# ginevracoal/robustBNNs

Measured on AMD Instinct MI355X. Metric: attack-samples/sec (test_pts x posterior_samples x PGD_iters), higher is better.
Workload: dtype f32 (full-width operands as three f16 pieces: 6 exact f16 MFMA product terms per fp32 product, f32 accumulate)

## Files before the change

robustbnns_amd/csrc/rbnn_triple.hip:

```cpp
#include "rbnn_common.hpp"
#include <algorithm>
#include <cstdlib>

namespace {

__device__ __forceinline__ void split3(float v, _Float16& p0, _Float16& p1, _Float16& p2) {
    p0 = (_Float16)v;
    float r = v - (float)p0;
    p1 = (_Float16)r;
    r -= (float)p1;
    p2 = (_Float16)r;
}

#ifndef RBNN_X3_PAIR_NOP
#define RBNN_X3_PAIR_NOP 0
#endif
#if RBNN_X3_PAIR_NOP
#define RBNN_X3_PAIR_PAD "\n\ts_nop 1"
#else
#define RBNN_X3_PAIR_PAD ""
#endif
#define RBNN_X3_PAIR_BODY \
    "v_bfe_i32 %[me], %[mw], %[b0], 1\n\t" \
    "v_bfe_i32 %[mo], %[mw], %[b1], 1\n\t" \
// ... 208 lines not shown
                if (k == 0 && ht + 1 < HTW) {
                    a0n = *(const f16x8*)(Wt + (ht + 1) * 3072);
                    a1n = *(const f16x8*)(Wt + (ht + 1) * 3072 + 1024);
                    a2n = *(const f16x8*)(Wt + (ht + 1) * 3072 + 2048);
                }
            }
            a0 = a0n; a1 = a1n; a2 = a2n;
        }
        {
            __builtin_amdgcn_sched_group_barrier(0x100, 3 * NTW + 3, 0);
#pragma unroll
            for (int ht = 0; ht < HTW; ++ht) {
                __builtin_amdgcn_sched_group_barrier(0x008, 3 * NTW, 0);
                if (ht + 1 < HTW) __builtin_amdgcn_sched_group_barrier(0x100, 3, 0);
                __builtin_amdgcn_sched_group_barrier(0x008, 3 * NTW, 0);
            }
        }
        if (!(RBNN_ABL & 2)) ring_wait_barrier<0>();
        const int hc0 = ch * BH;
        kt = wrap ? 0 : kt + 1;
        ch = wrap ? ch + 1 : ch;
        if (!wrap) continue;

        if (RBNN_ABL & 8) {
            float t = 0.f;
#pragma unroll
            for (int ht = 0; ht < HTW; ++ht)
#pragma unroll
                for (int nt = 0; nt < NTW; ++nt) { t += acc[ht][nt][0] + acc[ht][nt][1] + acc[ht][nt][2] + acc[ht][nt][3]; acc[ht][nt] = (f32x4){0.f, 0.f, 0.f, 0.f}; }
            if (t == 12345.678f) a.P[tid] = t;
            continue;
        }
        const int hw0 = hc0 + (wave_h * HTW) * 16;
        unsigned mine[NTW];
#pragma unroll
        for (int nt = 0; nt < NTW; ++nt) mine[nt] = 0u;
#pragma unroll
        for (int ht = 0; ht < HTW; ++ht) {
            const int hrow = hw0 + ht * 16 + 4 * lg;
            const f32x4 bias = *(const f32x4*)(a.b + (long long)sw * a.H + hrow);
            f32x4 w2f = (f32x4){0.f, 0.f, 0.f, 0.f};
            if (LAYER2 && li < a.C) w2f = *(const f32x4*)(a.W2 + ((long long)sw * a.C + li) * a.H + hrow);
#pragma unroll
            for (int nt = 0; nt < NTW; ++nt) {
                const int n = n0 + (wave_n * NTW + nt) * 16 + li;
                f32x4 v = acc[ht][nt] * out_scale + bias, hv;
                acc[ht][nt] = (f32x4){0.f, 0.f, 0.f, 0.f};
                unsigned bits = 0;
#pragma unroll
                for (int r = 0; r < 4; ++r) {
                    bits |= (v[r] > 0.f ? 1u : 0u) << r;
                    hv[r] = act_fwd<ACT>(v[r]);
                }
                if (BITMASK) {
                    unsigned part = bits << (16 * (ht & 1) + 4 * lg);
                    part |= __shfl_xor(part, 16);
                    part |= __shfl_xor(part, 32);
                    if (lg == (ht >> 1)) mine[nt] |= part;
                }
                if (!BITMASK && a.dact && n < a.N) {
                    f32x4 dv;
#pragma unroll
                    for (int r = 0; r < 4; ++r) dv[r] = act_grad_from_value<ACT>(hv[r]);
                    *(f32x4*)(a.dact + ((long long)s * a.N + n) * a.H + hrow) = dv;
                }
                if (LAYER2) {
#pragma unroll
                    for (int r = 0; r < 4; ++r) zacc[nt] = MFMA16(w2f[r], hv[r], zacc[nt]);
                } else {
#ifdef RBNN_X3_L1_ABL_NOSTORE
                    if (n < a.N && hv[0] == 1.2345e-30f) {
#else
                    if (n < a.N) {
#endif
                        const long long blk = ((long long)s * HW + (hrow >> 5)) * ((a.N + 15) >> 4) + (n >> 4);
#ifdef RBNN_X3_L1_ABL_SMALL
                        char* const row = a.hid + ((blk * 2048) & 0xFFC00) + (n & 15) * 128 + ((hrow >> 4) & 1) * 64 + lg * 16;
#else
                        char* const row = a.hid + blk * 2048 + (n & 15) * 128 + ((hrow >> 4) & 1) * 64 + lg * 16;
#endif
                        *(f32x4*)row = hv * hid_scale;
                    }
                }
            }
        }
        if (BITMASK && a.mask) {
#pragma unroll
            for (int nt = 0; nt < NTW; ++nt) {
                const int n = n0 + (wave_n * NTW + nt) * 16 + li;
                if (lg < HTW / 2 && n < a.N) a.mask[((long long)s * HW + (hw0 >> 5) + lg) * mask_ld(a.N) + n] = mine[nt];
            }
        }
    }
    if (RBNN_ABL & 2) ring_wait_barrier<0>();

    if (!LAYER2) return;
#pragma unroll
    for (int nt = 0; nt < NTW; ++nt)
        *(f32x4*)(zred + (wave_h * BN + (wave_n * NTW + nt) * 16 + li) * 16 + 4 * lg) = zacc[nt];
    __syncthreads();
    if (tid < BN) {
        const int n = n0 + tid;
        float z[16];
#pragma unroll
        for (int q = 0; q < 4; ++q) {
            f32x4 sum = *(const f32x4*)(zred + tid * 16 + 4 * q);
#pragma unroll
            for (int w = 1; w < WH; ++w) sum += *(const f32x4*)(zred + (w * BN + tid) * 16 + 4 * q);
#pragma unroll
            for (int r = 0; r < 4; ++r) z[4 * q + r] = sum[r];
        }
        float m = -INFINITY;
#pragma unroll
        for (int c = 0; c < 16; ++c) {
            if (c < a.C) { z[c] += a.b2[(long long)sw * a.C + c]; m = fmaxf(m, z[c]); }
            else z[c] = 0.f;
        }
        if (a.out_kind == RBNN_OUT_PROBS) {
            float den = 0.f;
#pragma unroll
            for (int c = 0; c < 16; ++c) if (c < a.C) { z[c] = expf(z[c] - m); den += z[c]; }
#pragma unroll
            for (int c = 0; c < 16; ++c) if (c < a.C) z[c] = z[c] / den;
        }
        if (n < a.N) {
            float* const dst = a.P + ((long long)s * a.N + n) * RBNN_CPAD;
#pragma unroll
            for (int q = 0; q < 4; ++q) *(f32x4*)(dst + 4 * q) = (f32x4){z[4 * q], z[4 * q + 1], z[4 * q + 2], z[4 * q + 3]};
        }
    }
}

template <int ACT, int WH, int HTW, int WN, int NTW, bool LAYER2, bool XF32>
int launch_forward_x3_cfg(FwdX3Args a, hipStream_t st) {
    constexpr int BH = WH * HTW * 16, BN = WN * NTW * 16;
    constexpr int LDSB = 2 * 3 * (BH + BN) * 64;
    static_assert(LDSB <= 160 * 1024, "LDS");
    a.NT = (a.N + BN - 1) / BN;
    auto kern = fc_forward_x3_kernel<ACT, WH, HTW, WN, NTW, LAYER2, XF32>;
    static unsigned long long attr_done = 0;
    if (!ensure_dynamic_lds((const void*)kern, LDSB, attr_done)) return RBNN_ERR_LAUNCH;
    const int grid = grid_for_items((long long)a.NT * a.S);
    hipLaunchKernelGGL(kern, dim3(grid), dim3(64 * WH * WN), LDSB, st, a);
    return launch_status();
}

template <int ACT, bool LAYER2, bool XF32>
int launch_forward_x3_act(const FwdX3Args& a, hipStream_t st) {
    if (a.H % 256 == 0) return launch_forward_x3_cfg<ACT, 4, 4, 2, 4, LAYER2, XF32>(a, st);
    if (a.H % 128 == 0) return launch_forward_x3_cfg<ACT, 2, 4, 2, 4, LAYER2, XF32>(a, st);
    return RBNN_ERR_UNSUPPORTED;
}

template <bool LAYER2, bool XF32 = false>
int launch_forward_x3(int act, const FwdX3Args& a, hipStream_t st) {
    switch (act) {
#ifndef RBNN_FAST_BUILD
        case RBNN_ACT_RELU:  return launch_forward_x3_act<RBNN_ACT_RELU, LAYER2, XF32>(a, st);
#endif
        case RBNN_ACT_LEAKY: return launch_forward_x3_act<RBNN_ACT_LEAKY, LAYER2, XF32>(a, st);
#ifndef RBNN_FAST_BUILD
        case RBNN_ACT_SIGM:  return launch_forward_x3_act<RBNN_ACT_SIGM, LAYER2, XF32>(a, st);
        case RBNN_ACT_TANH:  return launch_forward_x3_act<RBNN_ACT_TANH, LAYER2, XF32>(a, st);
#endif
    }
    return RBNN_ERR_UNSUPPORTED;
}

__global__ void triple_cols_kernel(const float* __restrict__ W, long long n_mats, int rows, int cols, int ld_src, float scale,
                                   uint4* __restrict__ dst, int ld_dst) {
    const long long i = (long long)blockIdx.x * blockDim.x + threadIdx.x;
    const int HB = rows / 32;
    if (i >= n_mats * HB * 4 * ld_dst) return;
    const int d = (int)(i % ld_dst);
    const int lg = (int)((i / ld_dst) % 4);
    const long long mh = i / (4LL * ld_dst);
    const long long m = mh / HB;
    const int hb = (int)(mh % HB);
    union { f16x8 v; uint4 u; } o[3];
#pragma unroll
    for (int j = 0; j < 8; ++j) {
        const int h = 32 * hb + 16 * (j >> 2) + 4 * lg + (j & 3);
        const float v = (d < cols) ? W[(m * rows + h) * ld_src + d] * scale : 0.f;
        _Float16 a, b, c;
        split3(v, a, b, c);
        o[0].v[j] = a; o[1].v[j] = b; o[2].v[j] = c;
    }
    const long long base = ((mh * 4 + lg) * 3) * ld_dst;
    dst[base + d] = o[0].u;
    dst[base + ld_dst + d] = o[1].u;
    dst[base + 2 * ld_dst + d] = o[2].u;
}

__global__ void triple_w2gen_kernel(const float* __restrict__ W2, int n_mats, int C, int H, float scale, uint4* __restrict__ dst) {
    const long long i = (long long)blockIdx.x * blockDim.x + threadIdx.x;
    if (i >= (long long)n_mats * (H / 16) * 128) return;
    const int lane = (int)(i & 63), li = lane & 15, lg = lane >> 4, k = (int)((i >> 6) & 1);
    const int t = (int)((i >> 7) % (H / 16));
    const long long m = (i >> 7) / (H / 16);
    _Float16 w[3][10];
#pragma unroll
    for (int c = 0; c < 10; ++c) {
        const float v = (c < C) ? W2[(m * C + c) * H + 16 * t + li] * scale : 0.f;
        split3(v, w[0][c], w[1][c], w[2][c]);
    }
    union { f16x8 v; uint4 u; } o;
    const _Float16 z = (_Float16)0.f;
    if (lg < 3) {
        const int piece = (k == 0) ? (lg == 2 ? 1 : 0) : (lg == 0 ? 1 : (lg == 1 ? 0 : 2));
#pragma unroll
        for (int j = 0; j < 8; ++j) o.v[j] = piece == 0 ? w[0][j] : (piece == 1 ? w[1][j] : w[2][j]);
    } else if (k == 0) {
        o.v[0] = w[0][8]; o.v[1] = w[0][9]; o.v[2] = w[0][8]; o.v[3] = w[0][9];
        o.v[4] = w[0][8]; o.v[5] = w[0][9]; o.v[6] = w[1][8]; o.v[7] = w[1][9];
    } else {
        o.v[0] = w[2][8]; o.v[1] = w[2][9]; o.v[2] = w[1][8]; o.v[3] = w[1][9];
        o.v[4] = z; o.v[5] = z; o.v[6] = z; o.v[7] = z;
    }
    dst[i] = o.u;
}

__host__ __device__ __forceinline__ int dz_swz3(long long n) { return (int)((0 - (n >> 2)) & 3); }

__global__ void __launch_bounds__(256) triple_dz_kernel(const float* __restrict__ dZ, int S, int N, long long N_pad, int C,
                                                        uint4* __restrict__ dst, float* __restrict__ gscale) {
    __shared__ float red[16][17];
    const int p = threadIdx.x & 15, q = threadIdx.x >> 4;
    const long long n = (long long)blockIdx.x * 16 + p;
    float m = 0.f;
    if (n < N)
        for (int s = q; s < S; s += 16) {
            const float* const src = dZ + ((long long)s * N + n) * RBNN_CPAD;
#pragma unroll
            for (int k = 0; k < 3; ++k) {
                const f32x4 v = *(const f32x4*)(src + 4 * k);
#pragma unroll
                for (int r = 0; r < 4; ++r) if (4 * k + r < C) m = fmaxf(m, fabsf(v[r]));
            }
        }
    red[q][p] = m;
    __syncthreads();
    m = 0.f;
#pragma unroll
    for (int i = 0; i < 16; ++i) m = fmaxf(m, red[i][p]);
    int e = 0;
    if (m > 0.f && m < INFINITY) e = min(13 - ilogbf(m), 120);
    if (q == 0) gscale[n] = ldexpf(1.f, -e);
    const int sw = dz_swz3(n);
    for (int s = q; s < S; s += 16) {
        _Float16 d[3][10];
        float v[12];
        if (n < N) {
            const float* const src = dZ + ((long long)s * N + n) * RBNN_CPAD;
#pragma unroll
            for (int k = 0; k < 3; ++k) {
                const f32x4 t = *(const f32x4*)(src + 4 * k);
#pragma unroll
                for (int r = 0; r < 4; ++r) v[4 * k + r] = t[r];
            }
        }
#pragma unroll
        for (int c = 0; c < 10; ++c) {
            const float x = (n < N && c < C) ? ldexpf(v[c], e) : 0.f;
            split3(x, d[0][c], d[1][c], d[2][c]);
        }
        uint4* const o = dst + ((long long)s * N_pad + n) * 4;
#pragma unroll
        for (int ch = 0; ch < 3; ++ch) {
            union { f16x8 v; uint4 u; } w;
#pragma unroll
            for (int j = 0; j < 8; ++j) w.v[j] = d[ch][j];
            o[ch ^ sw] = w.u;
        }
        union { f16x8 v; uint4 u; } t;
        t.v[0] = d[0][8]; t.v[1] = d[0][9]; t.v[2] = d[1][8]; t.v[3] = d[1][9];
        t.v[4] = d[2][8]; t.v[5] = d[2][9]; t.v[6] = d[0][8]; t.v[7] = d[0][9];
        o[3 ^ sw] = t.u;
    }
}

template <int MODE>
__device__ __forceinline__ void tail_dz(const float* __restrict__ prow, const float (&gmean)[16], int y, int C, float inv_S, float (&out)[16]) {
    float p[16], g[16];
#pragma unroll
    for (int q = 0; q < 4; ++q) {
        const f32x4 v = *(const f32x4*)(prow + 4 * q);
#pragma unroll
        for (int r = 0; r < 4; ++r) p[4 * q + r] = v[r];
    }
    if (MODE == RBNN_LOSS_PER_SAMPLE) {
        ce_softmax_grad<16>(p, C, y, inv_S, g);
    } else {
#pragma unroll
        for (int c = 0; c < 16; ++c) g[c] = gmean[c];
    }
    if (MODE == RBNN_LOSS_MEAN_LOGIT) {
#pragma unroll
        for (int c = 0; c < 16; ++c) out[c] = g[c];
    } else {
        softmax_backward<16>(g, p, C, out);
    }
}

template <int MODE>
__global__ void __launch_bounds__(256) step_tail_x3_kernel(const float* __restrict__ P, const int* __restrict__ labels, int S, float inv_S, int N,
                                                           long long N_pad, int C, float* __restrict__ Psum_out, int ldo,
                                                           uint4* __restrict__ dst, float* __restrict__ gscale) {
    __shared__ float red[16][17];
    __shared__ float psum[16][16];
    const int p = threadIdx.x & 15, q = threadIdx.x >> 4;
    const long long n = (long long)blockIdx.x * 16 + p;
    if (MODE != RBNN_LOSS_PER_SAMPLE) {
        if (q < 4) {
            f32x4 sum = (f32x4){0.f, 0.f, 0.f, 0.f};
            if (n < N)
                for (int s = 0; s < S; ++s) sum += *(const f32x4*)(P + ((long long)s * N + n) * RBNN_CPAD + 4 * q);
#pragma unroll
            for (int r = 0; r < 4; ++r) {
                psum[p][4 * q + r] = sum[r];
                if (Psum_out && n < N && 4 * q + r < C) Psum_out[n * ldo + 4 * q + r] = sum[r];
            }
        }
        __syncthreads();
    }
    const int y = (n < N) ? labels[n] : 0;
    float gmean[16];
    if (MODE != RBNN_LOSS_PER_SAMPLE) {
        float t[16];
#pragma unroll
        for (int c = 0; c < 16; ++c) t[c] = (c < C) ? psum[p][c] * inv_S : 0.f;
        ce_softmax_grad<16>(t, C, y, inv_S, gmean);
    } else {
#pragma unroll
        for (int c = 0; c < 16; ++c) gmean[c] = 0.f;
    }
    float m = 0.f;
    if (n < N)
        for (int s = q; s < S; s += 16) {
            float dz[16];
            tail_dz<MODE>(P + ((long long)s * N + n) * RBNN_CPAD, gmean, y, C, inv_S, dz);
#pragma unroll
            for (int c = 0; c < 12; ++c) if (c < C) m = fmaxf(m, fabsf(dz[c]));
        }
    red[q][p] = m;
    __syncthreads();
    m = 0.f;
#pragma unroll
    for (int i = 0; i < 16; ++i) m = fmaxf(m, red[i][p]);
    int e = 0;
    if (m > 0.f && m < INFINITY) e = min(13 - ilogbf(m), 120);
    if (q == 0) gscale[n] = ldexpf(1.f, -e);
    const int sw = dz_swz3(n);
    for (int s = q; s < S; s += 16) {
        _Float16 d[3][10];
        float dz[16];
#pragma unroll
        for (int c = 0; c < 16; ++c) dz[c] = 0.f;
        if (n < N) tail_dz<MODE>(P + ((long long)s * N + n) * RBNN_CPAD, gmean, y, C, inv_S, dz);
#pragma unroll
        for (int c = 0; c < 10; ++c) {
            const float x = (n < N && c < C) ? ldexpf(dz[c], e) : 0.f;
            split3(x, d[0][c], d[1][c], d[2][c]);
        }
        uint4* const o = dst + ((long long)s * N_pad + n) * 4;
#pragma unroll
        for (int ch = 0; ch < 3; ++ch) {
            union { f16x8 v; uint4 u; } w;
#pragma unroll
            for (int j = 0; j < 8; ++j) w.v[j] = d[ch][j];
            o[ch ^ sw] = w.u;
        }
        union { f16x8 v; uint4 u; } t;
        t.v[0] = d[0][8]; t.v[1] = d[0][9]; t.v[2] = d[1][8]; t.v[3] = d[1][9];
        t.v[4] = d[2][8]; t.v[5] = d[2][9]; t.v[6] = d[0][8]; t.v[7] = d[0][9];
        o[3 ^ sw] = t.u;
    }
}

__global__ void __launch_bounds__(256) attack_step_x3_kernel(float* __restrict__ X, const float* __restrict__ X0, int ldx, const float* __restrict__ G,
                                                             int K, long long slab_stride, int ldg, const float* __restrict__ alpha, float alpha_scalar,
                                                             float eps, int project, long long N, int D, const rbnn_dev_scale* __restrict__ ds,
                                                             uint4* __restrict__ dst, int groups) {
    const long long i = (long long)blockIdx.x * blockDim.x + threadIdx.x;
    if (i >= N * groups) return;
    const long long n = i / groups;
    const int gq = (int)(i % groups), d0 = 8 * gq;
    const float scale = ds->scale;
    float xn[8];
#pragma unroll
    for (int j = 0; j < 8; ++j) xn[j] = 0.f;
    if (d0 < D) {
        const float step = alpha ? alpha[n] : alpha_scalar;
#pragma unroll
        for (int h = 0; h < 2; ++h) {
            const int d = d0 + 4 * h;
            if (d < D) {
                f32x4 g = *(const f32x4*)(G + n * ldg + d);
                for (int k = 1; k < K; ++k) g += *(const f32x4*)(G + k * slab_stride + n * ldg + d);
                const f32x4 x = *(const f32x4*)(X + n * ldx + d);
                f32x4 x0 = x, out;
                if (project) x0 = *(const f32x4*)(X0 + n * ldx + d);
#pragma unroll
                for (int r = 0; r < 4; ++r) {
                    const float sgn = (g[r] > 0.f) ? 1.f : ((g[r] < 0.f) ? -1.f : 0.f);
                    float pert = x[r] + step * sgn;
                    if (project) pert = x0[r] + fminf(fmaxf(pert - x0[r], -eps), eps);
                    out[r] = fminf(fmaxf(pert, 0.f), 1.f);
                    xn[4 * h + r] = out[r];
                }
                *(f32x4*)(X + n * ldx + d) = out;
            }
        }
    }
    union { f16x8 v; uint4 u; } o[3];
#pragma unroll
    for (int j = 0; j < 8; ++j) {
        const float v = (d0 + j < D) ? xn[j] * scale : 0.f;
        _Float16 a, b, c;
        split3(v, a, b, c);
        o[0].v[j] = a; o[1].v[j] = b; o[2].v[j] = c;
    }
    uint4* const out = dst + (((n >> 4) * (groups >> 2) + (gq >> 2)) * 192 + (n & 15) * 4 + (gq & 3));
    out[0] = o[0].u; out[64] = o[1].u; out[128] = o[2].u;
}

#define GEN_Q3 (-17)

struct GradX3Args {
    const char* dzg;  long long n_pad;  const float* gscale;  const uint32_t* mask;
    const char* W1c;  int ldc;
    const char* W2g;
    int H;  int HW;  const int* sidx;  int S;  int chunk;  int nchunks;
    int N;  int NT;  int ND;  int Dt;
    float* out;  int ldo;  float out_scale;
    const uint32_t* omask;  int OHW;
    const float* amem;
    const float* dact;  const float* odact;
};
enum { X3_FC = 0, X3_FC2_STEP1 = 1, X3_FC2_STEP2 = 2 };

template <int ACT, int TD, int MODE>
__global__ void __launch_bounds__(256, 2) fc_grad_x3_kernel(const GradX3Args a) {
    constexpr int NW = 4;
    constexpr bool GEN = MODE != X3_FC2_STEP2;
    constexpr bool BITMASK = (ACT == RBNN_ACT_RELU || ACT == RBNN_ACT_LEAKY);
    constexpr bool STREAM = !GEN || !BITMASK;
    constexpr int NTW = 16 / NW, BM = 256, LD = TD * 16;
    constexpr int W1B = 12 * LD * 16;
    constexpr int NPIECE = W1B / 1024, PPW = (NPIECE + NW - 1) / NW;
    constexpr int BUFB = W1B + 4096 + 1024;
    constexpr int DZB = BM * 64;
    static_assert(W1B % 1024 == 0, "whole DMA pieces");
    extern __shared__ __attribute__((aligned(16))) float lds[];
    char* const ldsb = (char*)lds;
    char* const dzl = ldsb + 2 * BUFB;

    int id;
    if (!item_of_block(blockIdx.x, a.NT * a.ND * a.nchunks, id)) return;
    int ntile, dg, ch;
    grad_item(id, a.NT, a.ND, STREAM, ntile, dg, ch);
    const int tid = threadIdx.x, lane = tid & 63, li = lane & 15, lg = lane >> 4;
    const int wave = __builtin_amdgcn_readfirstlane(tid >> 6);
    const int nb = ntile * BM + wave * (NTW * 16);
    const int dc0 = dg * LD;
    const int Dp = a.Dt * 16;
    const int ntd = min(TD, a.Dt - dg * TD);
    const int s_begin = ch * a.chunk, s_end = min(a.S, s_begin + a.chunk);
    const int HS = a.H / 32, nst = (s_end - s_begin) * HS;

    unsigned goff[PPW];
#pragma unroll
    for (int i = 0; i < PPW; ++i) {
        const int f = (wave + NW * i) * 1024 + lane * 16, seg = f / (LD * 16), d = (f % (LD * 16)) >> 4;
        goff[i] = (unsigned)(seg * a.ldc + min(dc0 + d, a.ldc - 1)) * 16u;
    }
    const unsigned loff = (unsigned)lane * 16u;

    f32x4 acc[NTW][TD];
#pragma unroll
    for (int nt = 0; nt < NTW; ++nt)
#pragma unroll
        for (int dt = 0; dt < TD; ++dt) acc[nt][dt] = (f32x4){0.f, 0.f, 0.f, 0.f};

    auto dz_issue = [&](int s) {
        const char* const src = a.dzg + ((long long)s * a.n_pad + nb) * 64;
#pragma unroll
        for (int j = 0; j < NTW; ++j) glds16((const float*)(src + j * 1024 + loff), (float*)(dzl + wave * (NTW * 1024) + j * 1024));
    };
    constexpr int NDMA = GEN ? (BITMASK ? PPW + 2 : PPW + 1) : PPW;
    struct StageSrc { const char* W; const char* G; const char* M; char* B; };
    auto stage_src = [&](int st, int buf) {
        const int si = st / HS, hb = st % HS, s = s_begin + si;
        const int sw = a.sidx ? a.sidx[s] : s;
        StageSrc r;
        r.W = a.W1c + ((long long)sw * HS + hb) * 12 * a.ldc * 16;
        r.G = a.W2g + ((long long)sw * (a.H / 16) + 2 * hb) * 2048 + wave * 1024;
        r.M = (const char*)(a.mask + ((long long)s * a.HW + hb) * a.n_pad + ntile * BM);
        r.B = ldsb + buf * BUFB;
        return r;
    };
    auto issue_piece = [&](const StageSrc& q, int i) {
        if (i < PPW) {
            if (wave + NW * i < NPIECE) glds16((const float*)(q.W + goff[i < PPW ? i : 0]), (float*)(q.B + (wave + NW * i) * 1024));
        } else if (i == PPW) {
            glds16((const float*)(q.G + loff), (float*)(q.B + W1B + wave * 1024));
        } else if (BITMASK && i == PPW + 1) {
            if (wave == NW - 1) glds16((const float*)(q.M + loff), (float*)(q.B + W1B + 4096));
        }
    };

    if (GEN) dz_issue(s_begin);
    {
        const StageSrc q = stage_src(0, 0);
#pragma unroll
        for (int i = 0; i < NDMA; ++i) issue_piece(q, i);
    }
    f32x4 am[STREAM ? NTW : 1][2];
    auto load_a = [&](int st) {
        const int s = s_begin + st / HS, h0 = (st % HS) * 32;
        const float* const base = GEN ? a.dact : a.amem;
#pragma unroll
        for (int nt = 0; nt < (STREAM ? NTW : 0); ++nt) {
            const int n = min(nb + nt * 16 + li, a.N - 1);
            const float* const src = base + ((long long)s * a.N + n) * a.H + h0 + 4 * lg;
            am[nt][0] = *(const f32x4*)src;
            am[nt][1] = *(const f32x4*)(src + 16);
        }
    };
    if (STREAM) load_a(0);
    ring_wait_barrier<0>();
    const float c_pos = ldexpf(1.f, GEN_Q3);
    const unsigned cp_bits = __float_as_uint(c_pos);
    const unsigned cn_bits = (ACT == RBNN_ACT_RELU) ? 0u : __float_as_uint(LEAKY_SLOPE * ldexpf(1.f, GEN_Q3));
    const int dzc1 = (lg == 2 ? 0 : lg), dzc2 = (lg == 0 ? 1 : (lg == 1 ? 2 : (lg == 2 ? 0 : 3)));
    const int sz = dz_swz3(li);
    const char* const dzw = dzl + wave * (NTW * 1024) + li * 64;
    f16x8 da0[NTW], da1[NTW], da2[NTW];
    for (int st = 0; st < nst; ++st) {
        const int buf = st & 1, hb = st % HS;
        const bool more = !(RBNN_ABL & 1) && st + 1 < nst;
        const StageSrc q = stage_src(more ? st + 1 : st, buf ^ 1);
        const char* const B = ldsb + buf * BUFB;
        const bool gen_on = GEN && (!(RBNN_ABL & 16) || st == 0);
        if (!GEN) {
#pragma unroll
            for (int nt = 0; nt < (GEN ? 0 : NTW); ++nt) {
                union { f16x8 v; unsigned u[4]; } o0, o1, o2;
#pragma unroll
                for (int t = 0; t < 2; ++t) {
                    split3_plain_pair(am[nt][t][0], am[nt][t][1], 1.f, o0.u[2 * t], o1.u[2 * t], o2.u[2 * t]);
                    split3_plain_pair(am[nt][t][2], am[nt][t][3], 1.f, o0.u[2 * t + 1], o1.u[2 * t + 1], o2.u[2 * t + 1]);
                }
                da0[nt] = o0.v; da1[nt] = o1.v; da2[nt] = o2.v;
            }
        }
        if (more) {
#pragma unroll
            for (int i = 0; i < NDMA; ++i) issue_piece(q, i);
        }
        f32x4 dm[(GEN && STREAM) ? NTW : 1][2];
        if (GEN && STREAM) {
#pragma unroll
            for (int nt = 0; nt < ((GEN && STREAM) ? NTW : 0); ++nt) { dm[nt][0] = am[nt][0] * c_pos; dm[nt][1] = am[nt][1] * c_pos; }
        }
        if (STREAM && st + 1 < nst) load_a(st + 1);

        if (gen_on) {
            const f16x8 w00 = *(const f16x8*)(B + W1B + lane * 16);
            const f16x8 w01 = *(const f16x8*)(B + W1B + 1024 + lane * 16);
            const f16x8 w10 = *(const f16x8*)(B + W1B + 2048 + lane * 16);
            const f16x8 w11 = *(const f16x8*)(B + W1B + 3072 + lane * 16);
            const unsigned* const Mk = (const unsigned*)(B + W1B + 4096) + wave * (NTW * 16) + li;
#pragma unroll
            for (int nt = 0; nt < NTW; ++nt) {
                const f16x8 dz1 = *(const f16x8*)(dzw + nt * 1024 + ((dzc1 ^ sz) * 16));
                const f16x8 dz2 = *(const f16x8*)(dzw + nt * 1024 + ((dzc2 ^ sz) * 16));
                const f32x4 z = (f32x4){0.f, 0.f, 0.f, 0.f};
                const f32x4 g0 = MFMA_H(w01, dz2, MFMA_H(w00, dz1, z)), g1 = MFMA_H(w11, dz2, MFMA_H(w10, dz1, z));
                union { f16x8 v; unsigned u[4]; } o0, o1, o2;
                if constexpr (BITMASK) {
                    const unsigned mw = Mk[nt * 16] >> (4 * lg);
                    split3_pair<0, true>(g0[0], g0[1], mw, cp_bits, cn_bits, 1.f, o0.u[0], o1.u[0], o2.u[0]);
                    split3_pair<2, false>(g0[2], g0[3], mw, cp_bits, cn_bits, 1.f, o0.u[1], o1.u[1], o2.u[1]);
                    split3_pair<16, true>(g1[0], g1[1], mw, cp_bits, cn_bits, 1.f, o0.u[2], o1.u[2], o2.u[2]);
                    split3_pair<18, false>(g1[2], g1[3], mw, cp_bits, cn_bits, 1.f, o0.u[3], o1.u[3], o2.u[3]);
                } else {
                    constexpr int q = (GEN && STREAM) ? 1 : 0;
                    split3_pair_m<true>(g0[0], g0[1], dm[q * nt][0][0], dm[q * nt][0][1], 1.f, o0.u[0], o1.u[0], o2.u[0]);
                    split3_pair_m<false>(g0[2], g0[3], dm[q * nt][0][2], dm[q * nt][0][3], 1.f, o0.u[1], o1.u[1], o2.u[1]);
                    split3_pair_m<true>(g1[0], g1[1], dm[q * nt][1][0], dm[q * nt][1][1], 1.f, o0.u[2], o1.u[2], o2.u[2]);
                    split3_pair_m<false>(g1[2], g1[3], dm[q * nt][1][2], dm[q * nt][1][3], 1.f, o0.u[3], o1.u[3], o2.u[3]);
                }
                da0[nt] = o0.v; da1[nt] = o1.v; da2[nt] = o2.v;
            }
        }
        if (GEN && !(RBNN_ABL & 1) && hb == HS - 1 && st + 1 < nst) {
            asm volatile("" ::: "memory");
            __builtin_amdgcn_s_waitcnt(0xC07F);
            asm volatile("" ::: "memory");
            dz_issue(s_begin + st / HS + 1);
        }
        const char* const Bw = B + (lg * 3 * LD + li) * 16;
        f16x8 bb[2][3];
        bb[0][0] = *(const f16x8*)(Bw); bb[0][1] = *(const f16x8*)(Bw + LD * 16); bb[0][2] = *(const f16x8*)(Bw + 2 * LD * 16);
#pragma unroll
        for (int dt = 0; dt < TD; ++dt) {
            if (dt < ntd) {
                f16x8 (&bc)[3] = bb[dt & 1];
                if (dt + 1 < TD) {
                    f16x8 (&bn)[3] = bb[(dt + 1) & 1];
                    bn[0] = *(const f16x8*)(Bw + (dt + 1) * 256);
                    bn[1] = *(const f16x8*)(Bw + LD * 16 + (dt + 1) * 256);
                    bn[2] = *(const f16x8*)(Bw + 2 * LD * 16 + (dt + 1) * 256);
                }
#pragma unroll
                for (int nt = 0; nt < NTW; ++nt) acc[nt][dt] = MFMA_H(da0[nt], bc[2], acc[nt][dt]);
#pragma unroll
                for (int nt = 0; nt < NTW; ++nt) acc[nt][dt] = MFMA_H(da2[nt], bc[0], acc[nt][dt]);
#pragma unroll
                for (int nt = 0; nt < NTW; ++nt) acc[nt][dt] = MFMA_H(da1[nt], bc[1], acc[nt][dt]);
#pragma unroll
                for (int nt = 0; nt < NTW; ++nt) acc[nt][dt] = MFMA_H(da1[nt], bc[0], acc[nt][dt]);
#pragma unroll
                for (int nt = 0; nt < NTW; ++nt) acc[nt][dt] = MFMA_H(da0[nt], bc[1], acc[nt][dt]);
#pragma unroll
                for (int nt = 0; nt < NTW; ++nt) acc[nt][dt] = MFMA_H(da0[nt], bc[0], acc[nt][dt]);
            }
        }
        if (!(RBNN_ABL & 2)) ring_wait_barrier<0>();
    }
    if (RBNN_ABL & 2) ring_wait_barrier<0>();

    if (RBNN_ABL & 8) {
        float t = 0.f;
#pragma unroll
        for (int nt = 0; nt < NTW; ++nt)
#pragma unroll
            for (int dt = 0; dt < TD; ++dt) t += acc[nt][dt][0] + acc[nt][dt][1] + acc[nt][dt][2] + acc[nt][dt][3];
        if (t == 12345.678f) a.out[tid] = t;
        return;
    }
    constexpr int LDW = LD + 4, C4 = LD / 4, E4 = 16 * C4;
    static_assert(NW * 16 * LDW * 4 <= 2 * BUFB + DZB, "the waves' transposition tiles fit the loop buffers");
    float* const tw = (float*)ldsb + wave * (16 * LDW);
#pragma unroll
    for (int nt = 0; nt < NTW; ++nt) {
#pragma unroll
        for (int r = 0; r < 4; ++r) {
            const int n = nb + nt * 16 + 4 * lg + r;
            const float gs = (MODE == X3_FC2_STEP1) ? a.out_scale : (n < a.N ? a.gscale[n] : 0.f) * a.out_scale;
#pragma unroll
            for (int dt = 0; dt < TD; ++dt) tw[(4 * lg + r) * LDW + dt * 16 + li] = acc[nt][dt][r] * gs;
        }
#pragma unroll
        for (int i = 0; i < (E4 + 63) / 64; ++i) {
            const int e4 = i * 64 + lane, row = e4 / C4, c4 = e4 - row * C4;
            const int n = nb + nt * 16 + row, d = dc0 + 4 * c4;
            if (e4 < E4 && n < a.N && d < Dp) {
                f32x4 v = *(const f32x4*)(tw + row * LDW + 4 * c4);
                if (MODE == X3_FC2_STEP1) {
                    if (BITMASK) {
                        const unsigned w = a.omask[((long long)ch * a.OHW + (d >> 5)) * a.n_pad + n] >> (d & 31);
#pragma unroll
                        for (int k = 0; k < 4; ++k) v[k] = ((w >> k) & 1u) ? v[k] : (ACT == RBNN_ACT_RELU ? 0.f : v[k] * LEAKY_SLOPE);
                    } else {
                        v *= *(const f32x4*)(a.odact + ((long long)ch * a.N + n) * a.ldo + d);
                    }
                }
                *(f32x4*)(a.out + ((long long)ch * a.N + n) * a.ldo + d) = v;
            }
        }
    }
}

template <int ACT, int TD, int MODE>
int launch_grad_x3_cfg(GradX3Args a, hipStream_t st) {
    constexpr int LDSB = 2 * (12 * TD * 16 * 16 + 5120) + 256 * 64;
    static_assert(2 * LDSB <= 160 * 1024, "two blocks per CU");
    a.NT = (a.N + 255) / 256;
    a.ND = (a.Dt + TD - 1) / TD;
    auto kern = fc_grad_x3_kernel<ACT, TD, MODE>;
    static unsigned long long attr_done = 0;
    if (!ensure_dynamic_lds((const void*)kern, LDSB, attr_done)) return RBNN_ERR_LAUNCH;
    const int grid = grid_for_items((long long)a.NT * a.ND * a.nchunks);
    hipLaunchKernelGGL(kern, dim3(grid), dim3(256), LDSB, st, a);
    return launch_status();
}

inline bool x3_grad_td9() {
    static const bool on = [] { const char* e = getenv("RBNN_X3_GRAD_TD9"); return !e || e[0] != '0'; }();
    return on;
}

template <int ACT, int TD, int MODE>
bool x3_grad_two_blocks() {
    static int ok[64] = {0};
    int dev = 0;
    if (hipGetDevice(&dev) != hipSuccess || dev < 0 || dev >= 64) return false;
    if (!ok[dev]) {
        constexpr int LDSB = 2 * (12 * TD * 16 * 16 + 5120) + 256 * 64;
        auto kern = fc_grad_x3_kernel<ACT, TD, MODE>;
        static unsigned long long attr_done = 0;
        int nb = 0;
        const bool fine = ensure_dynamic_lds((const void*)kern, LDSB, attr_done) &&
                          hipOccupancyMaxActiveBlocksPerMultiprocessor(&nb, kern, 256, LDSB) == hipSuccess && nb >= 2;
        ok[dev] = fine ? 1 : 2;
    }
    return ok[dev] == 1;
}

template <int ACT, int MODE>
int launch_grad_x3(const GradX3Args& a, hipStream_t st) {
    if constexpr (MODE == X3_FC && (ACT == RBNN_ACT_RELU || ACT == RBNN_ACT_LEAKY)) {
        if (x3_grad_td9() && (a.Dt + 8) / 9 < (a.Dt + 6) / 7 && x3_grad_two_blocks<ACT, 9, MODE>()) return launch_grad_x3_cfg<ACT, 9, MODE>(a, st);
    }
    if constexpr (MODE != X3_FC2_STEP2 && (ACT == RBNN_ACT_RELU || ACT == RBNN_ACT_LEAKY)) {
        if (x3_grad_td9() && (a.Dt + 7) / 8 < (a.Dt + 6) / 7 && x3_grad_two_blocks<ACT, 8, MODE>()) return launch_grad_x3_cfg<ACT, 8, MODE>(a, st);
    }
    if ((a.Dt + 6) / 7 < (a.Dt + 3) / 4) return launch_grad_x3_cfg<ACT, 7, MODE>(a, st);
    return launch_grad_x3_cfg<ACT, 4, MODE>(a, st);
}

template <int MODE>
int launch_grad_x3_act(int act, const GradX3Args& a, hipStream_t st) {
#ifndef RBNN_FAST_BUILD
    if (act == RBNN_ACT_RELU) return launch_grad_x3<RBNN_ACT_RELU, MODE>(a, st);
    if (act == RBNN_ACT_SIGM || act == RBNN_ACT_TANH) return launch_grad_x3<RBNN_ACT_SIGM, MODE>(a, st);
#endif
    return launch_grad_x3<RBNN_ACT_LEAKY, MODE>(a, st);
}

}

extern "C" {

static int triple_rows_launch(const float* src, int64_t rows, int32_t cols, int32_t ld_src, int32_t scale_exp,
                              const rbnn_dev_scale* dev_scale, void* dst, int32_t ld_dst, void* stream, int grouped) {
    if (!src || !dst) return RBNN_ERR_NULL;
    if (rows < 1 || cols < 1 || ld_src < cols || ld_dst < cols || (ld_dst & 31)) return RBNN_ERR_SHAPE;
    if (scale_exp < -100 || scale_exp > 100) return RBNN_ERR_SHAPE;
    if (!aligned16(dst)) return RBNN_ERR_ALIGN;
    const int groups = ld_dst / 8;
    const long long total = (long long)rows * groups;
    hipLaunchKernelGGL(triple_rows_kernel, dim3((unsigned)((total + 255) / 256)), dim3(256), 0, (hipStream_t)stream,
                       src, (long long)rows, cols, ld_src, ldexpf(1.f, scale_exp), dev_scale, (uint4*)dst, groups, grouped);
    return launch_status();
}

int rbnn_triple_rows(const float* src, int64_t rows, int32_t cols, int32_t ld_src, int32_t scale_exp,
                     const rbnn_dev_scale* dev_scale, void* dst, int32_t ld_dst, void* stream) {
    return triple_rows_launch(src, rows, cols, ld_src, scale_exp, dev_scale, dst, ld_dst, stream, 0);
}

int rbnn_triple_rows_grouped(const float* src, int64_t rows, int32_t cols, int32_t ld_src, int32_t scale_exp,
                             const rbnn_dev_scale* dev_scale, void* dst, int32_t ld_dst, void* stream) {
    return triple_rows_launch(src, rows, cols, ld_src, scale_exp, dev_scale, dst, ld_dst, stream, 1);
}

int rbnn_triple_cols(const float* W, int64_t n_mats, int32_t rows, int32_t cols, int32_t ld_src, int32_t scale_exp,
                     void* dst, int32_t ld_dst, void* stream) {
    if (!W || !dst) return RBNN_ERR_NULL;
    if (n_mats < 1 || rows < 32 || (rows & 31) || cols < 1 || ld_src < cols || ld_dst < cols || (ld_dst & 15)) return RBNN_ERR_SHAPE;
    if (scale_exp < -100 || scale_exp > 100) return RBNN_ERR_SHAPE;
    if (!aligned16(dst)) return RBNN_ERR_ALIGN;
    const long long total = (long long)n_mats * (rows / 32) * 4 * ld_dst;
    hipLaunchKernelGGL(triple_cols_kernel, dim3((unsigned)((total + 255) / 256)), dim3(256), 0, (hipStream_t)stream,
                       W, (long long)n_mats, rows, cols, ld_src, ldexpf(1.f, scale_exp), (uint4*)dst, ld_dst);
    return launch_status();
}

int rbnn_triple_w2gen(const float* W2, int32_t n_mats, int32_t C, int32_t H, int32_t scale_exp, void* dst, void* stream) {
    if (!W2 || !dst) return RBNN_ERR_NULL;
    if (n_mats < 1 || C < 1 || C > 10 || H < 16 || (H & 15)) return RBNN_ERR_SHAPE;
    if (scale_exp < -100 || scale_exp > 100) return RBNN_ERR_SHAPE;
    if (!aligned16(dst)) return RBNN_ERR_ALIGN;
    const long long total = (long long)n_mats * (H / 16) * 128;
    hipLaunchKernelGGL(triple_w2gen_kernel, dim3((unsigned)((total + 255) / 256)), dim3(256), 0, (hipStream_t)stream,
                       W2, n_mats, C, H, ldexpf(1.f, scale_exp), (uint4*)dst);
    return launch_status();
}

int rbnn_triple_workspace_query(const rbnn_posterior* net, const rbnn_triple_images* tp, int32_t N, int32_t S,
                                rbnn_triple_workspace_sizes* out) {
    if (!net || !tp || !out) return RBNN_ERR_NULL;
    if (N < 1 || S < 1 || tp->ld_rows < net->in_features || (tp->ld_rows & 31)) return RBNN_ERR_SHAPE;
    rbnn_triple_workspace_sizes z = {};
    z.X_triple = (size_t)((N + 15) / 16 * 16) * tp->ld_rows * 6;
    z.dZ_gen = (size_t)S * mask_ld(N) * 64;
    z.g_scale = (size_t)mask_ld(N) * sizeof(float);
    z.hid_triple = net->arch == RBNN_ARCH_FC2 ? (size_t)S * ((N + 15) / 16 * 16) * net->hidden * 4 : 0;
    *out = z;
    return RBNN_OK;
}

int rbnn_fc_forward_triple(const rbnn_posterior* net, const rbnn_triple_images* tp, const rbnn_triple_workspace* tws,
                           int32_t x_exp, const rbnn_dev_scale* dev_scales, int32_t N, const int32_t* sidx, int32_t S,
                           int32_t out_kind, const rbnn_workspace* ws, void* stream) {
    if (!net || !tp || !tws || !tws->X_triple || !ws || !ws->P || !tp->W1_rows) return RBNN_ERR_NULL;
    if (!net->b1 || !net->W2 || !net->b2) return RBNN_ERR_NULL;
    if (net->arch != RBNN_ARCH_FC && net->arch != RBNN_ARCH_FC2) return RBNN_ERR_UNSUPPORTED;
    if (net->activation < RBNN_ACT_RELU || net->activation > RBNN_ACT_TANH) return RBNN_ERR_UNSUPPORTED;
    const bool fc2 = net->arch == RBNN_ARCH_FC2, bm = net->activation == RBNN_ACT_RELU || net->activation == RBNN_ACT_LEAKY;
    const int H = net->hidden, ld = tp->ld_rows;
    if (H < 128 || (H % 128) || ld < net->in_features || (ld & 31)) return RBNN_ERR_SHAPE;
    if (net->n_classes < 1 || net->n_classes > RBNN_CPAD || N < 1 || S < 1) return RBNN_ERR_SHAPE;
    if ((long long)H * ld * 6 >= (1LL << 32) || ((long long)N + 15) * ld * 6 >= (1LL << 32) || ((long long)N + 15) * H * 6 >= (1LL << 32)) return RBNN_ERR_SHAPE;
    if (out_kind != RBNN_OUT_PROBS && out_kind != RBNN_OUT_LOGITS) return RBNN_ERR_UNSUPPORTED;
    if (!aligned16(tws->X_triple) || !aligned16(tp->W1_rows) || !aligned16(ws->P) || !aligned16(net->b1) || !aligned16(net->W2)) return RBNN_ERR_ALIGN;
    if (fc2 && (!tp->Wm_rows || !net->bm || !tws->hid_triple || (bm ? !ws->mask2 : !ws->dact2))) return RBNN_ERR_NULL;
    if (fc2 && (!aligned16(tp->Wm_rows) || !aligned16(tws->hid_triple) || !aligned16(net->bm))) return RBNN_ERR_ALIGN;
    hipStream_t st = (hipStream_t)stream;
    FwdX3Args a = {};
    a.X = (const char*)tws->X_triple; a.ldx = ld; a.N = N; a.x_sample_bytes = 0; a.x_group_bytes = (unsigned)(ld / 32) * 3072u; a.x_stage_bytes = 3072u;
    a.W = (const char*)tp->W1_rows; a.w_sample_bytes = (long long)H * ld * 6; a.ldw = ld; a.KT = ld / 32;
    a.b = net->b1; a.W2 = net->W2; a.b2 = net->b2; a.C = net->n_classes; a.H = H;
    a.sidx = sidx; a.S = S; a.out_scale = ldexpf(1.f, -((dev_scales ? 0 : x_exp) + tp->w1_exp)); a.x_ds = dev_scales;
    a.P = ws->P; a.mask = ws->mask1; a.dact = ws->dact1; a.out_kind = out_kind;
    if (!fc2) return launch_forward_x3<true>(net->activation, a, st);
    a.hid = (char*)tws->hid_triple; a.hid_scale = ldexpf(1.f, tp->h1_exp); a.hid_ds = dev_scales ? dev_scales + 1 : nullptr;
    int rc = launch_forward_x3<false>(net->activation, a, st);
    if (rc) return rc;
    FwdX3Args b = a;
    const int NG = (N + 15) / 16;
    b.X = (const char*)tws->hid_triple; b.ldx = H; b.x_sample_bytes = (long long)NG * 16 * H * 4; b.x_group_bytes = 2048u; b.x_stage_bytes = (unsigned)NG * 2048u;
    b.W = (const char*)tp->Wm_rows; b.w_sample_bytes = (long long)H * H * 6; b.ldw = H; b.KT = H / 32;
    b.b = net->bm; b.out_scale = ldexpf(1.f, -((dev_scales ? 0 : tp->h1_exp) + tp->wm_exp));
    b.x_ds = dev_scales ? dev_scales + 1 : nullptr; b.hid_ds = nullptr;
    b.mask = ws->mask2; b.dact = ws->dact2; b.hid = nullptr;
    return launch_forward_x3<true, true>(net->activation, b, st);
}

int rbnn_step_tail_triple(int32_t mode, const float* P, const int32_t* labels, int32_t S, float inv_S, int32_t N, int32_t C, float* Psum_out,
                          int32_t ldo, const rbnn_triple_workspace* tws, void* stream) {
    if (!P || !labels || !tws || !tws->dZ_gen || !tws->g_scale) return RBNN_ERR_NULL;
    if (mode != RBNN_LOSS_MEAN_PROB && mode != RBNN_LOSS_PER_SAMPLE && mode != RBNN_LOSS_MEAN_LOGIT) return RBNN_ERR_UNSUPPORTED;
    if (S < 1 || N < 1 || C < 1 || C > 10 || (Psum_out && ldo < C)) return RBNN_ERR_SHAPE;
    if (!aligned16(P) || !aligned16(tws->dZ_gen)) return RBNN_ERR_ALIGN;
    const long long n_pad = mask_ld(N);
    const dim3 grid((unsigned)(n_pad / 16)), block(256);
    hipStream_t st = (hipStream_t)stream;
    if (mode == RBNN_LOSS_MEAN_PROB)
        hipLaunchKernelGGL(step_tail_x3_kernel<RBNN_LOSS_MEAN_PROB>, grid, block, 0, st, P, labels, S, inv_S, N, n_pad, C, Psum_out, ldo, (uint4*)tws->dZ_gen, tws->g_scale);
    else if (mode == RBNN_LOSS_PER_SAMPLE)
        hipLaunchKernelGGL(step_tail_x3_kernel<RBNN_LOSS_PER_SAMPLE>, grid, block, 0, st, P, labels, S, inv_S, N, n_pad, C, Psum_out, ldo, (uint4*)tws->dZ_gen, tws->g_scale);
    else
        hipLaunchKernelGGL(step_tail_x3_kernel<RBNN_LOSS_MEAN_LOGIT>, grid, block, 0, st, P, labels, S, inv_S, N, n_pad, C, Psum_out, ldo, (uint4*)tws->dZ_gen, tws->g_scale);
    return launch_status();
}

int rbnn_attack_step_triple(float* X, const float* X0, int32_t ldx, const float* G, int32_t K, size_t slab_stride, int32_t ldg, const float* alpha,
                            float alpha_scalar, float eps, int32_t project, int32_t N, int32_t D, const rbnn_dev_scale* dev_scale, void* X_triple,
                            int32_t ld_rows, void* stream) {
    if (!X || !G || (project && !X0) || !dev_scale || !X_triple) return RBNN_ERR_NULL;
    if (N < 1 || D < 1 || ldx < D || ldg < D || K < 1 || ld_rows < D || (ld_rows & 31)) return RBNN_ERR_SHAPE;
    if ((D & 3) || (ldx & 3) || (ldg & 3) || (slab_stride & 3)) return RBNN_ERR_SHAPE;
    if (!aligned16(X) || !aligned16(G) || (project && !aligned16(X0)) || !aligned16(X_triple)) return RBNN_ERR_ALIGN;
    const int groups = ld_rows / 8;
    const long long total = (long long)N * groups;
    hipLaunchKernelGGL(attack_step_x3_kernel, dim3((unsigned)((total + 255) / 256)), dim3(256), 0, (hipStream_t)stream,
                       X, X0, ldx, G, K, (long long)slab_stride, ldg, alpha, alpha_scalar, eps, project, (long long)N, D, dev_scale, (uint4*)X_triple, groups);
    return launch_status();
}

int rbnn_fc_input_grad_triple(const rbnn_posterior* net, const rbnn_triple_images* tp, const int32_t* sidx, int32_t S,
                              int32_t N, int32_t chunk, const rbnn_workspace* ws, const rbnn_triple_workspace* tws,
                              int32_t* n_slabs_out, void* stream) {
    if (!net || !tp || !ws || !tws || !ws->slabs) return RBNN_ERR_NULL;
    if (!tp->W1_cols || !tp->W2_gen || !tws->dZ_gen || !tws->g_scale) return RBNN_ERR_NULL;
    if (net->arch != RBNN_ARCH_FC && net->arch != RBNN_ARCH_FC2) return RBNN_ERR_UNSUPPORTED;
    if (net->activation < RBNN_ACT_RELU || net->activation > RBNN_ACT_TANH) return RBNN_ERR_UNSUPPORTED;
    const bool fc2 = net->arch == RBNN_ARCH_FC2, bm = net->activation == RBNN_ACT_RELU || net->activation == RBNN_ACT_LEAKY;
    if (bm ? !ws->mask1 : !ws->dact1) return RBNN_ERR_NULL;
    if (fc2 && (bm ? !ws->mask2 : !ws->dact2)) return RBNN_ERR_NULL;
    const int H = net->hidden, Dp = net->in_stride, C = net->n_classes;
    if (H < 128 || (H % 128) || C < 1 || C > 10 || N < 1 || S < 1) return RBNN_ERR_SHAPE;
    if (tp->ld_cols != Dp || (Dp & 15)) return RBNN_ERR_SHAPE;
    if (!aligned16(tp->W1_cols) || !aligned16(tp->W2_gen) || !aligned16(tws->dZ_gen) || (ws->dZ && !aligned16(ws->dZ))) return RBNN_ERR_ALIGN;
    if (fc2 && (!tp->Wm_cols || !ws->dhid1)) return RBNN_ERR_NULL;
    if (fc2 && (!aligned16(tp->Wm_cols) || !aligned16(ws->dhid1))) return RBNN_ERR_ALIGN;
    hipStream_t st = (hipStream_t)stream;
    if (chunk <= 0) {
        rbnn_workspace_sizes q;
        const int rc = rbnn_workspace_query(net, N, S, 0, &q);
        if (rc) return rc;
        chunk = q.chunk;
    }
    if (chunk > S) chunk = S;
    const int nchunks = (S + chunk - 1) / chunk;
    if (n_slabs_out) *n_slabs_out = nchunks;
    const long long n_pad = mask_ld(N);
    if (ws->dZ) {
        hipLaunchKernelGGL(triple_dz_kernel, dim3((unsigned)(n_pad / 16)), dim3(256), 0, st,
                           ws->dZ, S, N, n_pad, C, (uint4*)tws->dZ_gen, tws->g_scale);
        if (hipGetLastError() != hipSuccess) return RBNN_ERR_LAUNCH;
    }
    GradX3Args g = {};
    g.dzg = (const char*)tws->dZ_gen; g.n_pad = n_pad; g.gscale = tws->g_scale;
    g.W2g = (const char*)tp->W2_gen;
    g.H = H; g.HW = H / 32; g.sidx = sidx; g.S = S; g.N = N;
    if (!fc2) {
        g.mask = ws->mask1; g.dact = ws->dact1; g.W1c = (const char*)tp->W1_cols; g.ldc = tp->ld_cols; g.Dt = Dp / 16;
        g.chunk = chunk; g.nchunks = nchunks; g.out = ws->slabs; g.ldo = Dp;
        g.out_scale = ldexpf(1.f, -(tp->w2_exp + GEN_Q3 + tp->w1_exp));
        return launch_grad_x3_act<X3_FC>(net->activation, g, st);
    }
    int q2 = 14;
    while ((1 << (q2 - 14)) < H) ++q2;
    g.mask = ws->mask2; g.dact = ws->dact2; g.odact = ws->dact1; g.W1c = (const char*)tp->Wm_cols; g.ldc = H; g.Dt = H / 16;
    g.chunk = 1; g.nchunks = S; g.out = ws->dhid1; g.ldo = H; g.out_scale = ldexpf(1.f, -q2);
    g.omask = ws->mask1; g.OHW = H / 32;
    int rc = launch_grad_x3_act<X3_FC2_STEP1>(net->activation, g, st);
    if (rc) return rc;
    GradX3Args h = g;
    h.amem = ws->dhid1; h.W1c = (const char*)tp->W1_cols; h.ldc = tp->ld_cols; h.Dt = Dp / 16;
    h.chunk = chunk; h.nchunks = nchunks; h.out = ws->slabs; h.ldo = Dp;
    h.out_scale = ldexpf(1.f, -(tp->w2_exp + GEN_Q3 + tp->wm_exp - q2 + tp->w1_exp));
    return launch_grad_x3_act<X3_FC2_STEP2>(net->activation, h, st);
}

}
```

Before: 135.7 million.

## Spread step-tail sample reduction over more threads with staged shared-memory sums

The step-tail kernel now handles 4 points per block instead of 16, giving 64 sample lanes per point and four times as many blocks. The mean-probability sum, which used to be a serial loop over all samples in 64 threads, is now loaded cooperatively by all 256 threads in chunks of 64 samples, staged in shared memory, and then summed. The aim is more parallelism and memory-level concurrency in this latency-bound tail. The cost is extra barriers and shared-memory traffic, and each block now writes narrower per-point output tiles.

```diff
diff --git a/robustbnns_amd/csrc/rbnn_triple.hip b/robustbnns_amd/csrc/rbnn_triple.hip
--- a/robustbnns_amd/csrc/rbnn_triple.hip
+++ b/robustbnns_amd/csrc/rbnn_triple.hip
@@ -534,19 +534,40 @@
     }
 }
 
+#define TAIL_PTS 4
+#define TAIL_SB 64
 template <int MODE>
 __global__ void __launch_bounds__(256) step_tail_x3_kernel(const float* __restrict__ P, const int* __restrict__ labels, int S, float inv_S, int N,
                                                            long long N_pad, int C, float* __restrict__ Psum_out, int ldo,
                                                            uint4* __restrict__ dst, float* __restrict__ gscale) {
-    __shared__ float red[16][17];
-    __shared__ float psum[16][16];
-    const int p = threadIdx.x & 15, q = threadIdx.x >> 4;
-    const long long n = (long long)blockIdx.x * 16 + p;
+    constexpr int PTS = TAIL_PTS, Q = 256 / PTS;
+    static_assert(PTS == 4, "the staging pass maps a thread to (sample, point, class quad) = (tid / 16, tid / 4 % 4, tid % 4)");
+    __shared__ float red[Q][PTS + 1];
+    __shared__ float psum[PTS][16];
+    __shared__ f32x4 stage[TAIL_SB][PTS][4];
+    const int p = threadIdx.x % PTS, q = threadIdx.x / PTS;
+    const long long n = (long long)blockIdx.x * PTS + p;
     if (MODE != RBNN_LOSS_PER_SAMPLE) {
+        const int sl = threadIdx.x >> 4, lp = (threadIdx.x >> 2) & 3, lq = threadIdx.x & 3;
+        const long long ln = (long long)blockIdx.x * PTS + lp;
+        f32x4 sum = (f32x4){0.f, 0.f, 0.f, 0.f};
+        for (int s0 = 0; s0 < S; s0 += TAIL_SB) {
+            f32x4 v[TAIL_SB / 16];
+#pragma unroll
+            for (int k = 0; k < TAIL_SB / 16; ++k) {
+                const int s = s0 + sl + 16 * k;
+                v[k] = (s < S && ln < N) ? *(const f32x4*)(P + ((long long)s * N + ln) * RBNN_CPAD + 4 * lq) : (f32x4){0.f, 0.f, 0.f, 0.f};
+            }
+#pragma unroll
+            for (int k = 0; k < TAIL_SB / 16; ++k) stage[sl + 16 * k][lp][lq] = v[k];
+            __syncthreads();
+            if (q < 4 && n < N) {
+                const int cnt = min(TAIL_SB, S - s0);
+                for (int i = 0; i < cnt; ++i) sum += stage[i][p][q];
+            }
+            __syncthreads();
+        }
         if (q < 4) {
-            f32x4 sum = (f32x4){0.f, 0.f, 0.f, 0.f};
-            if (n < N)
-                for (int s = 0; s < S; ++s) sum += *(const f32x4*)(P + ((long long)s * N + n) * RBNN_CPAD + 4 * q);
 #pragma unroll
             for (int r = 0; r < 4; ++r) {
                 psum[p][4 * q + r] = sum[r];
@@ -568,7 +589,7 @@
     }
     float m = 0.f;
     if (n < N)
-        for (int s = q; s < S; s += 16) {
+        for (int s = q; s < S; s += Q) {
             float dz[16];
             tail_dz<MODE>(P + ((long long)s * N + n) * RBNN_CPAD, gmean, y, C, inv_S, dz);
 #pragma unroll
@@ -578,12 +599,12 @@
     __syncthreads();
     m = 0.f;
 #pragma unroll
-    for (int i = 0; i < 16; ++i) m = fmaxf(m, red[i][p]);
+    for (int i = 0; i < Q; ++i) m = fmaxf(m, red[i][p]);
     int e = 0;
     if (m > 0.f && m < INFINITY) e = min(13 - ilogbf(m), 120);
     if (q == 0) gscale[n] = ldexpf(1.f, -e);
     const int sw = dz_swz3(n);
-    for (int s = q; s < S; s += 16) {
+    for (int s = q; s < S; s += Q) {
         _Float16 d[3][10];
         float dz[16];
 #pragma unroll
@@ -1069,7 +1090,7 @@
     if (S < 1 || N < 1 || C < 1 || C > 10 || (Psum_out && ldo < C)) return RBNN_ERR_SHAPE;
     if (!aligned16(P) || !aligned16(tws->dZ_gen)) return RBNN_ERR_ALIGN;
     const long long n_pad = mask_ld(N);
-    const dim3 grid((unsigned)(n_pad / 16)), block(256);
+    const dim3 grid((unsigned)(n_pad / TAIL_PTS)), block(256);
     hipStream_t st = (hipStream_t)stream;
     if (mode == RBNN_LOSS_MEAN_PROB)
         hipLaunchKernelGGL(step_tail_x3_kernel<RBNN_LOSS_MEAN_PROB>, grid, block, 0, st, P, labels, S, inv_S, N, n_pad, C, Psum_out, ldo, (uint4*)tws->dZ_gen, tws->g_scale);
```

Result: no change. 136.4 million (median of 6 runs) (+0.5%).
